# RaduAlexandru/permuto_sdf

Measured on AMD Instinct MI355X. Metric: ray-samples/sec (encode+MLP+composite), higher is better.
Workload: dtype f32 (MLP products on 2 fp16 operand pieces per fp32 value, fp32 accumulation; the 3-piece / 24-bit figure is value_fp32_equivalent_24bit)

## Files before the change

include/psdf.h:

```cpp
#ifndef PSDF_H
#define PSDF_H
#include <stdint.h>
#ifdef __cplusplus
extern "C" {
#endif

int64_t psdf_encode_convention(int which);
int psdf_encode_set_conventions(uint32_t hash_multiplier, int rank_tie_raises_later);

int psdf_encode_forward(int pos_dim, int nr_feat, int64_t N, int nr_levels, int capacity, const float* positions,
    const float* lattice, const float* scale_factor, const float* shifts, const float* window, int concat_points,
    float points_scaling, float* sliced, void* stream);

int psdf_encode_forward_mark(int pos_dim, int nr_feat, int64_t N, int nr_levels, int capacity, const float* positions,
    const float* lattice, const float* scale_factor, const float* shifts, const float* window, int concat_points,
    float points_scaling, float* sliced, unsigned char* touched_blocks, int block_rows_log2, void* stream);

int psdf_encode_backward(int pos_dim, int nr_feat, int64_t N, int nr_levels, int capacity, const float* positions,
    const float* lattice, const float* scale_factor, const float* shifts, const float* window, int concat_points,
    float points_scaling, const float* grad_sliced, float* grad_lattice, float* grad_positions, void* stream);

int64_t psdf_encode_backward_workspace_bytes(int pos_dim, int nr_feat, int64_t N, int nr_levels, int capacity);
int psdf_encode_backward_ws(int pos_dim, int nr_feat, int64_t N, int nr_levels, int capacity, const float* positions,
    const float* lattice, const float* scale_factor, const float* shifts, const float* window, int concat_points,
    float points_scaling, const float* grad_sliced, float* grad_lattice, float* grad_positions, void* workspace,
    int64_t workspace_bytes, void* stream);
int psdf_encode_backward_level_shares(int* counts, int max_levels);


int psdf_encode_double_backward(int pos_dim, int nr_feat, int64_t N, int nr_levels, int capacity, const float*
    positions, const float* lattice, const float* scale_factor, const float* shifts, const float* window, int
    concat_points, float points_scaling, const float* dd_positions, const float* grad_sliced, float* grad_lattice,
    float* grad_grad_sliced, void* stream);
int psdf_encode_double_backward_ws(int pos_dim, int nr_feat, int64_t N, int nr_levels, int capacity, const float* positions,
                                   const float* lattice, const float* scale_factor, const float* shifts, const float* window,
                                   int concat_points, float points_scaling, const float* dd_positions, const float* grad_sliced,
                                   float* grad_lattice, float* grad_grad_sliced, const float* grad_sliced_direct,
                                   void* workspace, int64_t workspace_bytes, void* stream);

int psdf_mlp_pack_f16(int n_layers, const int* dims, const float* const* weights, const float* const* biases, float* packed,
    void* stream);
int psdf_mlp_forward_f16(int n_layers, const int* dims, int64_t N, const float* X, const float* packed, float* Y, void* stream);

int psdf_mlp_forward_set_form(int waves);
int psdf_mlp_forward_last_form(void);

int psdf_neus_composite_forward(int nr_rays, const int* start_end, int equal, int fixed, int max_nr_samples, const float* sdf,
    const float* dirs, const float* gradients, const float* dt, const float* rgb, const float* inv_s, float cos_anneal_ratio,
    float* pred, float* bg, float* weights, void* stream);
int psdf_neus_composite_backward(int nr_rays, const int* start_end, int equal, int fixed, int max_nr_samples, int max_per_ray,
    const float* grad_pred, const float* grad_bg, const float* sdf, const float* dirs, const float* gradients, const float* dt,
    const float* rgb, const float* inv_s, float cos_anneal_ratio, int reference_compat, float* grad_sdf, float* grad_gradients,
    float* grad_rgb, float* grad_inv_s, void* stream);

int psdf_nerf_composite_forward(int nr_rays, const int* start_end, int equal, int fixed, int max_nr_samples, const float* raw_density,
                                const float* dt, const float* rgb, const float* fg_pred, const float* fg_bg, float* pred_bg,
                                float* pred, void* stream);
int psdf_nerf_composite_backward(int nr_rays, const int* start_end, int equal, int fixed, int max_nr_samples, int max_per_ray,
                                 const float* grad_pred, const float* fg_bg, const float* raw_density, const float* dt,
                                 const float* rgb, int reference_compat, float* grad_raw_density, float* grad_rgb,
                                 float* grad_fg_bg, void* stream);

int psdf_last_path(int family);
enum {
  PSDF_MLP_OP_FORWARD = 0,
  PSDF_MLP_OP_FORWARD_F16 = 1,
  PSDF_MLP_OP_FORWARD_WIDE_F16 = 2,
  PSDF_MLP_OP_BACKWARD = 3,
  PSDF_MLP_OP_BACKWARD_DATA = 4,
  PSDF_MLP_OP_BACKWARD_DATA_MASKED = 5,
  PSDF_MLP_OP_DOUBLE_BACKWARD = 6,
  PSDF_MLP_OP_DOUBLE_BACKWARD_PLUS = 7
};
int psdf_mlp_supported(int op, int n_layers, const int* dims);

int psdf_mlp_backward_split(int n_layers, const int* dims, int64_t N, const float* X, const float* const* weights,
    const float* const* biases, const float* dY, float* dX, float* const* dW, float* const* db, void* stream);

int psdf_mlp_backward_split_f16(int n_layers, const int* dims, int64_t N, const float* X, const float* const* weights,
    const float* const* biases, const float* dY, float* dX, float* const* dW, float* const* db, void* stream);
int psdf_mlp_backward_split_f16_form(void);
unsigned psdf_mlp_f16_range_events(void);

int psdf_mlp_forward_wide_f16(int n_layers, const int* dims, int64_t N, const float* X, const float* const* weights,
    const float* const* biases, float* Y, void* stream);
int psdf_mlp_backward_wide_form(void);
int psdf_mlp_backward_wide(int n_layers, const int* dims, int64_t N, const float* X, const float* const* weights,
    const float* const* biases, const float* dY, float* dX, float* const* dW, float* const* db, void* stream);

int psdf_lipshitz_normalize_forward(int out, int in, const float* W, const float* c, float* Wn, void* stream);
int psdf_lipshitz_normalize_backward(int out, int in, const float* W, const float* c, const float* grad_Wn, float* grad_W,
    float* grad_c, void* stream);
int psdf_lipshitz_normalize_forward_multi(int n_layers, const int* out, const int* in, const float* const* W, const float* const* c,
                                          float* const* Wn, void* stream);
int psdf_lipshitz_normalize_backward_multi(int n_layers, const int* out, const int* in, const float* const* W, const float* const* c,
                                           const float* const* grad_Wn, float* const* grad_W, float* const* grad_c, void* stream);

int psdf_neus_alpha_forward(int64_t N, const float* sdf, const float* dirs, const float* gradients, const float* dt,
    const float* inv_s, float cos_anneal_ratio, float* alpha, float* one_minus_alpha, void* stream);
int psdf_neus_alpha_backward(int64_t N, const float* grad_alpha, const float* sdf, const float* dirs, const float*
    gradients, const float* dt, const float* inv_s, float cos_anneal_ratio, float* grad_sdf, float* grad_gradients,
    float* grad_inv_s, void* stream);
int psdf_l1_loss(int64_t R, int C, const float* pred, const float* gt, const unsigned char* mask, float scale,
    float* loss, float* grad_pred, void* stream);
int psdf_eikonal_loss(int64_t N, const float* gradients, float scale, float* loss, float* grad_gradients, void* stream);
int psdf_normalize3(int64_t N, const float* x, const float* grad_y, float* out, void* stream);
int psdf_sigmoid_rows(int64_t N, int C, const float* x_fm, float* y, void* stream);
int psdf_sigmoid_rows_backward(int64_t N, int C, const float* grad_y, const float* y, float* grad_x_fm, void* stream);
int psdf_curvature_shift(int64_t N, const float* points, const float* gradients, const float* rand_directions, float
    epsilon, const float* grad_shifted, float* out, void* stream);
int psdf_curvature_loss(int64_t N, const float* gradients, const float* gradients_shifted, float scale, float* loss,
    float* grad_gradients, float* grad_gradients_shifted, void* stream);
int psdf_offsurface_loss(int64_t N, const float* sdf, float sharpness, float scale, float* loss, float* grad_sdf, void*
    stream);
int psdf_nerf_alpha_forward(int64_t N, const float* raw_density, const float* dt, float* alpha, float* one_minus_alpha,
    void* stream);
int psdf_nerf_alpha_backward(int64_t N, const float* raw_density, const float* dt, const float* grad_alpha, const float*
    grad_one_minus_alpha, float* grad_raw_density, void* stream);

int64_t psdf_mlp_packed_size(int n_layers, const int* dims);

int psdf_mlp_pack(int n_layers, const int* dims, const float* const* weights, const float* const* biases, float*
    packed, void* stream);

int psdf_mlp_forward(int n_layers, const int* dims, int64_t N, const float* X, const float* packed, float* Y, void*
    stream);

int psdf_encode_forward_masked(int pos_dim, int nr_feat, int64_t N, int nr_levels, int capacity, const float* positions,
    const float* lattice, const float* scale_factor, const float* shifts, const float* window, int concat_points, float
    points_scaling, const uint8_t* skip, float* sliced, void* stream);
int psdf_mlp_forward_masked(int n_layers, const int* dims, int64_t N, const float* X, const float* packed, const uint8_t*
    skip, float* Y, void* stream);
int psdf_mlp_backward_data_masked(int n_layers, const int* dims, int64_t N, const float* X, const float* const* weights,
    const float* const* biases, const float* dY, const uint8_t* skip, float* dX, void* stream);
int psdf_encode_backward_positions_masked(int pos_dim, int nr_feat, int64_t N, int nr_levels, int capacity, const float*
    positions, const float* lattice, const float* scale_factor, const float* shifts, const float* window, int
    concat_points, float points_scaling, const float* grad_sliced, const uint8_t* skip, float* grad_positions, void*
    stream);

int psdf_mlp_backward(int n_layers, const int* dims, int64_t N, const float* X, const float* const* weights, const
    float* const* biases, const float* dY, float* dX, float* const* dW, float* const* db, void* stream);

int psdf_mlp_double_backward(int n_layers, const int* dims, int64_t N, const float* X, const float* const* weights,
    const float* const* biases, const float* dY, const float* V, float* dX2, float* const* dW, float* const* db,
    void* stream);
int psdf_mlp_double_backward_plus(int n_layers, const int* dims, int64_t N, const float* X, const float* const* weights,
    const float* const* biases, const float* dY, const float* V, const float* dY2, float* dX2, float* const* dW,
    float* const* db, void* stream);

int psdf_encode_mlp_forward(int64_t N, int nr_levels, int capacity, const float* positions, const float* lattice,
    const float* scale_factor, const float* shifts, const float* window, int concat_points, float points_scaling,
    int n_layers, const int* dims, const float* packed, const uint8_t* skip, float* feat, float* Y, void* stream);

int psdf_adamw_step(int64_t n, float* param, const float* grad, float* exp_avg, float* exp_avg_sq, float lr, float
    beta1, float beta2, float eps, float weight_decay, int step, float grad_scale, void* stream);

int psdf_adamw_step_multi(int n_tensors, const int64_t* sizes, float* const* params, const float* const* grads, float*
    const* exp_avgs, float* const* exp_avg_sqs, float lr, float beta1, float beta2, float eps, float weight_decay, int
    step, float grad_scale, void* stream);

int psdf_adamw_step_blocks(int64_t n_blocks, int block_elems, float* param, float* grad, float* exp_avg, float*
// ... 193 lines not shown
```

permuto_sdf_amd/csrc/encode.hip:

```cpp
#include <cstdio>
#include <cstring>
#include <mutex>
#include <type_traits>
#include <vector>

#include "encode_device.h"
#include "encode_plan.h"

namespace {

template <int P, int F, bool PLAIN = false>
__global__ void __launch_bounds__(PSDF_BLOCK)
    encode_fwd_kernel(int64_t N, int L, uint32_t capacity, EncConv conv, const float* __restrict__ positions,
                      const float* __restrict__ lattice, const float* __restrict__ scale_factor,
                      const float* __restrict__ shifts, const float* __restrict__ window, float points_scaling,
                      int pad_points, const unsigned char* __restrict__ skip, float* __restrict__ sliced,
                      unsigned char* __restrict__ touched, int touch_shift, int blocks_per_level) {
  const int level = blockIdx.y;
  const int64_t ntiles = (N + PSDF_BLOCK - 1) / PSDF_BLOCK;
  for (int64_t tile = blockIdx.x; tile < ntiles; tile += gridDim.x) {
  const int64_t n = tile * PSDF_BLOCK + threadIdx.x;
  if (n >= N) continue;
  if (!PLAIN && skip && skip[n]) continue;
  float pos[P];
  load_pos<P>(positions, n, pos);
  if (level >= L) {
    const int e = level - L;
#pragma unroll
    for (int f = 0; f < F; f++) {
      const int d = e * F + f;
      float v = 0.f;
#pragma unroll
      for (int i = 0; i < P; i++)
        if (i == d) v = pos[i] * points_scaling;
      if (d < P || pad_points) sliced[((int64_t)level * F + f) * N + n] = v;
    }
    continue;
  }
  const float w = window[level];
  if (w == 0.f) {
#pragma unroll
    for (int f = 0; f < F; f++) sliced[((int64_t)level * F + f) * N + n] = 0.f;
    continue;
  }
  Simplex<P> s;
  compute_simplex<P>(pos, shifts + level * P, scale_factor + level * P, s, conv.tie_later);
  const float* __restrict__ table = lattice + (int64_t)level * capacity * F;
  uint32_t row[P + 1];
  vertex_rows<P>(s, capacity, row, conv.hash_c);
  if (!PLAIN && touched) {
#pragma unroll
    for (int r = 0; r <= P; r++) touched[(int64_t)level * blocks_per_level + (row[r] >> touch_shift)] = 1;
  }
  float fv[P + 1][F];
#pragma unroll
  for (int r = 0; r <= P; r++) {
    const char* tb = reinterpret_cast<const char*>(table);
    if (F == 2) {
      float2 t = *reinterpret_cast<const float2*>(tb + (row[r] * 8u));
      fv[r][0] = t.x;
      fv[r][F - 1] = t.y;
    } else {
#pragma unroll
      for (int f = 0; f < F; f++) fv[r][f] = *reinterpret_cast<const float*>(tb + (row[r] * (uint32_t)(F * 4) + (uint32_t)(f * 4)));
    }
  }
  float acc[F];
#pragma unroll
  for (int r = 0; r <= P; r++) {
    const float bw = s.bary[r] * w;
#pragma unroll
    for (int f = 0; f < F; f++) acc[f] = r == 0 ? fv[r][f] * bw : acc[f] + fv[r][f] * bw;
  }
#pragma unroll
  for (int f = 0; f < F; f++) sliced[((int64_t)level * F + f) * N + n] = acc[f];
  }
}


constexpr uint32_t SC_EMPTY = 0xFFFFFFFFu;
constexpr uint32_t Q_NONE = 0xFFFFFFFFu;
#if !defined(PSDF_ENC_QSPT)
#define PSDF_ENC_QSPT 2
#endif
constexpr int QUEUE_SPT = PSDF_ENC_QSPT;

__device__ __forceinline__ void lds_add_pair(float* p, float a, float b, int& hot) {
  if (hot == 0) {
    unsigned long long* q = reinterpret_cast<unsigned long long*>(p);
    unsigned long long old = *q;
#pragma unroll
    for (int it = 0; it < 4; it++) {
      const float x = __uint_as_float((uint32_t)old) + a;
      const float y = __uint_as_float((uint32_t)(old >> 32)) + b;
      const unsigned long long want = (unsigned long long)__float_as_uint(x) | ((unsigned long long)__float_as_uint(y) << 32);
      const unsigned long long prev = atomicCAS(q, old, want);
      if (prev == old) return;
      old = prev;
    }
    hot = 8;
  } else {
    hot--;
  }
  atomicAdd(p, a);
  atomicAdd(p + 1, b);
}

template <int F>
__device__ __forceinline__ bool combine_runs16(uint32_t key, float (&v)[F]) {
  constexpr int ROW_SHR = 0x110, ROW_SHL = 0x100;
  const int k = (int)key;
  const int kprev = __builtin_amdgcn_update_dpp(0, k, ROW_SHR | 1, 0xf, 0xf, true);
  const float joined = (kprev == k) ? 1.0f : 0.0f;
  float j = joined;
#define PSDF_SCAN_STEP(D)                                                                                        \
  {                                                                                                              \
    _Pragma("unroll") for (int i = 0; i < F; i++) v[i] = __builtin_fmaf(                                         \
        __int_as_float(__builtin_amdgcn_update_dpp(0, __float_as_int(v[i]), ROW_SHR | D, 0xf, 0xf, true)), j, v[i]); \
    j = j * __int_as_float(__builtin_amdgcn_update_dpp(0, __float_as_int(j), ROW_SHR | D, 0xf, 0xf, true));      \
  }
  PSDF_SCAN_STEP(1)
  PSDF_SCAN_STEP(2)
  PSDF_SCAN_STEP(4)
  PSDF_SCAN_STEP(8)
#undef PSDF_SCAN_STEP
  const int next_joined = __builtin_amdgcn_update_dpp(0, __float_as_int(joined), ROW_SHL | 1, 0xf, 0xf, true);
  return key != Q_NONE && next_joined == 0;
}

template <int F, int TOTAL = 8192>
struct ScatterCache {
  static constexpr int SC_SLOTS = TOTAL / F;
  uint32_t* tags;
  float* sums;
  int* stats;
  __device__ __forceinline__ void init(float* lds) {
    tags = reinterpret_cast<uint32_t*>(lds);
    sums = lds + SC_SLOTS;
    stats = reinterpret_cast<int*>(lds + SC_SLOTS + SC_SLOTS * F);
    for (int i = threadIdx.x; i < SC_SLOTS; i += blockDim.x) tags[i] = SC_EMPTY;
    for (int i = threadIdx.x; i < SC_SLOTS * F; i += blockDim.x) sums[i] = 0.f;
    if (threadIdx.x == 0) {
      stats[0] = 0;
      stats[1] = 0;
      stats[2] = 1;
    }
    __syncthreads();
  }
  __device__ __forceinline__ int add(uint32_t row, const float* v, int& hot) {
    const uint32_t slot = (row ^ (row >> 12)) & (SC_SLOTS - 1);
    uint32_t old = tags[slot];
    if (old == SC_EMPTY) old = atomicCAS(&tags[slot], SC_EMPTY, row);
    if (old == SC_EMPTY || old == row) {
      static_assert(F % 2 == 0, "pairs");
#pragma unroll
      for (int f = 0; f < F; f += 2) lds_add_pair(&sums[slot * F + f], v[f], v[f + 1], hot);
      return old == row ? 2 : 1;
    }
    return 0;
  }
  __device__ __forceinline__ void flush(float* __restrict__ table_grad) {
    __syncthreads();
    for (int i = threadIdx.x; i < SC_SLOTS; i += blockDim.x) {
      const uint32_t row = tags[i];
      if (row != SC_EMPTY) {
#pragma unroll
        for (int f = 0; f < F; f++) {
          const float v = sums[i * F + f];
          if (v != 0.f) atomicAdd(table_grad + (int64_t)row * F + f, v);
        }
      }
    }
  }
  static constexpr size_t bytes() { return (size_t)(SC_SLOTS + SC_SLOTS * F + 4) * 4; }
};

template <typename SC>
__device__ __forceinline__ bool cache_vote(SC& sc, int hits, int tries) {
  hits = (int)psdf::wave_sum((float)hits);
  tries = (int)psdf::wave_sum((float)tries);
  if (psdf::lane_id() == 0) {
    atomicAdd(&sc.stats[0], hits);
    atomicAdd(&sc.stats[1], tries);
  }
  __syncthreads();
  return sc.stats[0] * 8 >= sc.stats[1];
}

struct Queues {
  uint16_t* rows;
  float* vals;
  int* tails;
  int cap, np, shift;
};
using psdf::enc_plan::Q_MAX_PARTS;
constexpr int Q_LDS_INTS = 4 * Q_MAX_PARTS + 4;

struct LevelQueues {
  char* rows;
  char* vals;
  uint32_t mask;
};
template <int F>
__device__ __forceinline__ LevelQueues level_queues(const Queues& Q, int level) {
  const int64_t e = (int64_t)level * Q.np * Q.cap;
  return LevelQueues{reinterpret_cast<char*>(Q.rows + e), reinterpret_cast<char*>(Q.vals + e * F), (1u << Q.shift) - 1u};
}
template <int F>
__device__ __forceinline__ void queue_store(const LevelQueues& LQ, uint32_t o, uint32_t row, const float* v) {
  *reinterpret_cast<uint16_t*>(LQ.rows + (o * 2u)) = (uint16_t)(row & LQ.mask);
  if (F == 2) {
    *reinterpret_cast<float2*>(LQ.vals + (o * 8u)) = make_float2(v[0], v[F - 1]);
  } else {
#pragma unroll
    for (int f = 0; f < F; f++) *reinterpret_cast<float*>(LQ.vals + (o * (uint32_t)(F * 4) + (uint32_t)(f * 4))) = v[f];
  }
}

template <int NC, int F>
__device__ __forceinline__ void queue_push(const Queues& Q, int level, int* q_cnt, int* q_base,
                                           const uint32_t (&crow)[NC], const float (&cval)[NC][F],
                                           float* __restrict__ table_grad) {
  int* q_aux = q_base + Q_MAX_PARTS;
  const LevelQueues LQ = level_queues<F>(Q, level);
  if (threadIdx.x < Q.np) q_cnt[threadIdx.x] = 0;
  __syncthreads();
  int slot[NC];
#pragma unroll
// ... 578 lines not shown
  float sfl[P], shl[P];
#pragma unroll
  for (int i = 0; i < P; i++) {
    sfl[i] = scale_factor[level * P + i];
    shl[i] = shifts[level * P + i];
  }
  for (int64_t tile = blockIdx.x; tile < ntiles; tile += gridDim.x, iter++) {
    const int64_t n = tile * PSDF_BLOCK + threadIdx.x;
    if (n < N) {
      float u[P], pos[P];
      load_pos<P>(dd_positions, n, u);
      load_pos<P>(positions, n, pos);
      Simplex<P> s;
      compute_simplex<P>(pos, shl, sfl, s, conv.tie_later);
      float aE[P + 1];
#pragma unroll
      for (int j = 0; j <= P; j++) aE[j] = 0.f;
#pragma unroll
      for (int k = 0; k < P; k++) {
        const float us = u[k] * sfl[k];
#pragma unroll
        for (int j = 0; j <= k; j++) aE[j] = aE[j] + us;
        aE[k + 1] = aE[k + 1] - us * (float)(k + 1);
      }
      float q[P + 2];
#pragma unroll
      for (int k = 0; k <= P + 1; k++) q[k] = 0.f;
      const float invp = 1.0f / (P + 1);
#pragma unroll
      for (int i = 0; i <= P; i++) {
        const float t = aE[i] * invp;
#pragma unroll
        for (int k = 0; k <= P + 1; k++) {
          if (k == P - s.rank[i]) q[k] = q[k] + t;
          if (k == P + 1 - s.rank[i]) q[k] = q[k] - t;
        }
      }
      q[0] = q[0] + q[P + 1];
      float g[F], gg[F];
#pragma unroll
      for (int f = 0; f < F; f++) {
        g[f] = grad_sliced[((int64_t)level * F + f) * N + n];
        gg[f] = 0.f;
      }
      uint32_t rows[P + 1];
      vertex_rows<P>(s, capacity, rows, conv.hash_c);
#pragma unroll
      for (int r = 0; r <= P; r++) {
        const uint32_t row = rows[r];
        const float qw = q[r] * w;
        if (LATTICE) {
          float v[F];
#pragma unroll
          for (int f = 0; f < F; f++) v[f] = qw * g[f];
          bool absorbed = false;
          if (use_cache) {
            const int rc = sc.add(row, v, hot);
            absorbed = rc != 0;
            hits += (rc == 2);
            tries++;
          }
          if (!absorbed) {
#pragma unroll
            for (int f = 0; f < F; f++) atomicAdd(grad_lattice + tbase + (int64_t)row * F + f, v[f]);
          }
        }
#pragma unroll
        for (int f = 0; f < F; f++) gg[f] = gg[f] + qw * lattice[tbase + (int64_t)row * F + f];
      }
#pragma unroll
      for (int f = 0; f < F; f++) grad_grad_sliced[((int64_t)level * F + f) * N + n] = gg[f];
    }
    if (LATTICE && iter == 0) use_cache = cache_vote(sc, hits, tries);
  }
  if (LATTICE) sc.flush(grad_lattice + tbase);
}

inline int extra_levels(int P, int F, int concat) { return concat ? (P + F - 1) / F : 0; }
inline int pad_points(int concat) { return concat == PSDF_ENC_CONCAT_PSEUDO_LEVELS; }
inline bool concat_ok(int concat) { return concat >= PSDF_ENC_CONCAT_NONE && concat <= PSDF_ENC_CONCAT_APPEND; }

}

namespace psdf {
EncConv& enc_conv_state() {
  static EncConv c{(uint32_t)PSDF_ENC_HASH_MULTIPLIER, (uint32_t)PSDF_ENC_RANK_TIE_RAISES_LATER};
  return c;
}
}

namespace {
namespace plan = psdf::enc_plan;
using plan::env_int;
template <int V>
using int_c = std::integral_constant<int, V>;

template <class Fn>
int dispatch_pf(int pos_dim, int nr_feat, Fn&& fn) {
  if (pos_dim == 3 && nr_feat == 2) return fn(int_c<3>{}, int_c<2>{});
  if (pos_dim == 4 && nr_feat == 2) return fn(int_c<4>{}, int_c<2>{});
  if (pos_dim == 2 && nr_feat == 2) return fn(int_c<2>{}, int_c<2>{});
  if (pos_dim == 3 && nr_feat == 4) return fn(int_c<3>{}, int_c<4>{});
  return PSDF_ERR_UNSUPPORTED;
}

struct EncCall {
  int64_t N;
  int nr_levels, Lt, capacity;
  const float *positions, *lattice, *scale_factor, *shifts, *window;
  float points_scaling;
  int pad;
  hipStream_t stream;
};

bool enc_call(EncCall& c, int pos_dim, int nr_feat, int64_t N, int nr_levels, int capacity, const float* positions,
              const float* lattice, const float* scale_factor, const float* shifts, const float* window, int concat_points,
              float points_scaling, void* stream) {
  if (N < 0 || nr_levels <= 0 || capacity <= 0 || !positions || !lattice || !concat_ok(concat_points)) return false;
  c = EncCall{N, nr_levels, nr_levels + extra_levels(pos_dim, nr_feat, concat_points), capacity, positions, lattice,
              scale_factor, shifts, window, points_scaling, pad_points(concat_points), (hipStream_t)stream};
  return true;
}

template <class Kernel, class... Rest>
void launch_enc(Kernel kern, dim3 grid, size_t shm, const EncCall& c, Rest... rest) {
  hipLaunchKernelGGL(kern, grid, dim3(PSDF_BLOCK), shm, c.stream, c.N, c.nr_levels, (uint32_t)c.capacity, psdf::enc_conv_state(),
                     c.positions, c.lattice, c.scale_factor, c.shifts, c.window, c.points_scaling, rest...);
}

int launched(int rc) {
  if (rc != PSDF_OK) return rc;
  PSDF_LAUNCH_CHECK();
  return PSDF_OK;
}

int device_cus() {
  static int cus[64] = {};
  int dev = 0;
  if (hipGetDevice(&dev) != hipSuccess || dev < 0 || dev >= 64) return 256;
  if (cus[dev] == 0) {
    int n = 0;
    if (hipDeviceGetAttribute(&n, hipDeviceAttributeMultiprocessorCount, dev) != hipSuccess || n <= 0) n = 256;
    cus[dev] = n;
  }
  return cus[dev];
}

dim3 plain_grid(const EncCall& c) {
  static const int wg_cap_env = env_int("PSDF_ENC_BWD_WG_PER_LEVEL", 0);
  const unsigned wg_cap = wg_cap_env > 0 ? (unsigned)wg_cap_env : 512u, nb = psdf_blocks(c.N, PSDF_BLOCK);
  return dim3(nb < wg_cap ? nb : wg_cap, c.Lt);
}

template <int P, int F>
int launch_fwd(int_c<P>, int_c<F>, const EncCall& c, dim3 grid, const unsigned char* skip, float* sliced, unsigned char* touched,
               int touch_shift) {
  const int touch_blocks = (c.capacity + (1 << touch_shift) - 1) >> touch_shift;
  if (!skip && !touched)
    launch_enc(encode_fwd_kernel<P, F, true>, grid, 0, c, c.pad, skip, sliced, touched, touch_shift, touch_blocks);
  else
    launch_enc(encode_fwd_kernel<P, F, false>, grid, 0, c, c.pad, skip, sliced, touched, touch_shift, touch_blocks);
  return PSDF_OK;
}

int encode_forward_impl(int pos_dim, int nr_feat, int64_t N, int nr_levels, int capacity, const float* positions,
                        const float* lattice, const float* scale_factor, const float* shifts, const float* window,
                        int concat_points, float points_scaling, const unsigned char* skip, float* sliced, void* stream,
                        unsigned char* touched = nullptr, int touch_shift = 0) {
  EncCall c;
  if (N == 0) return PSDF_OK;
  if (!enc_call(c, pos_dim, nr_feat, N, nr_levels, capacity, positions, lattice, scale_factor, shifts, window, concat_points,
                points_scaling, stream) || !sliced)
    return PSDF_ERR_ARG;
  if ((int64_t)capacity * nr_feat * 4 > 0xffffffffll) return PSDF_ERR_UNSUPPORTED;
  dim3 grid(psdf_blocks(N, PSDF_BLOCK), c.Lt);
  static const int fwd_env = env_int("PSDF_ENC_FWD_WGS", -1);
  const int fwd_wgs = fwd_env >= 0 ? fwd_env : device_cus() * 8;
  if (fwd_wgs > 0 && (int)grid.x > fwd_wgs) grid.x = fwd_wgs;
  return launched(dispatch_pf(pos_dim, nr_feat, [&](auto p, auto f) {
    return launch_fwd(p, f, c, grid, skip, sliced, touched, touch_shift);
  }));
}

template <int P, int F, int POS_LPB>
void launch_bwd_pos_lpb(const EncCall& c, const float* grad_sliced, const unsigned char* skip, float* grad_positions, bool capturing) {
  static const bool force_atomics = env_int("PSDF_ENC_POS_ATOMICS", 0) != 0;
  const int groups = (c.Lt + POS_LPB - 1) / POS_LPB;
  static const size_t slab_cap = (size_t)plan::env_long("PSDF_ENC_POS_SLAB_MAX_MB", 256) << 20;
  const size_t slab_bytes = (size_t)groups * c.N * P * sizeof(float);
  const bool use_slabs = groups > 1 && !force_atomics && !capturing && slab_bytes <= slab_cap;
  float* slabs = use_slabs ? (float*)psdf::stream_scratch(slab_bytes, c.stream) : nullptr;
  const auto pos_kernel = [&](auto kern, float* out) {
    hipLaunchKernelGGL(kern, dim3(psdf_blocks(c.N, PSDF_BLOCK), groups), dim3(PSDF_BLOCK), 0, c.stream, c.N, c.nr_levels, c.Lt,
                       (uint32_t)c.capacity, psdf::enc_conv_state(), c.positions, c.lattice, c.scale_factor, c.shifts, c.window,
                       c.points_scaling, c.pad, grad_sliced, skip, out);
  };
  if (slabs) {
    pos_kernel(encode_bwd_pos_kernel<P, F, true, POS_LPB>, slabs);
    hipLaunchKernelGGL(encode_bwd_pos_reduce_kernel, dim3(psdf_blocks(c.N * P, PSDF_BLOCK)), dim3(PSDF_BLOCK), 0, c.stream,
                       c.N * P, P, groups, slabs, skip, grad_positions);
  } else {
    pos_kernel(encode_bwd_pos_kernel<P, F, false, POS_LPB>, grad_positions);
  }
}

template <int P, int F>
int launch_bwd_pos(int_c<P>, int_c<F>, const EncCall& c, const float* grad_sliced, const unsigned char* skip, float* grad_positions) {
  const bool capturing = psdf::stream_scratch(16, c.stream) == nullptr;
  if (capturing)
    launch_bwd_pos_lpb<P, F, 4>(c, grad_sliced, skip, grad_positions, true);
  else if (c.N >= ((int64_t)1 << 17))
    launch_bwd_pos_lpb<P, F, 2>(c, grad_sliced, skip, grad_positions, false);
  else
    launch_bwd_pos_lpb<P, F, 8>(c, grad_sliced, skip, grad_positions, false);
  return PSDF_OK;
}

plan::QueuePlan queue_plan(int pos_dim, int nr_feat, int64_t N, int nr_levels, int capacity) {
  static const int64_t min_n = plan::env_long("PSDF_ENC_QUEUE_MIN_N", (int64_t)1 << 13);
  static const int delta = env_int("PSDF_ENC_QUEUE_SLICE_LOG2_DELTA", 1);
  return plan::queue_plan(pos_dim, nr_feat, N, nr_levels, capacity, min_n, delta);
}
Queues queue_carve(void* ws, const plan::QueuePlan& p) {
  char* b = (char*)ws;
  return Queues{(uint16_t*)b, (float*)(b + p.rows_bytes), (int*)(b + p.rows_bytes + p.vals_bytes), p.cap, p.np, p.shift};
}
bool queue_begin(int pos_dim, int nr_feat, const EncCall& c, bool wanted, void* ws, int64_t ws_bytes, size_t also_zeroed, Queues& Q,
                 hipError_t& e) {
  const plan::QueuePlan p = (wanted && ws) ? queue_plan(pos_dim, nr_feat, c.N, c.nr_levels, c.capacity) : plan::QueuePlan{};
  if (p.bytes == 0 || ws_bytes < p.bytes) return false;
  Q = queue_carve(ws, p);
  e = hipMemsetAsync(Q.tails, 0, (size_t)c.nr_levels * Q.np * sizeof(int) + also_zeroed, c.stream);
  return true;
}

struct EncBalance {
  int levels = 0, total = 0, kind = 0, bucket = -1;
  const void* ident = nullptr;
  uint32_t gen = 0;
  uint64_t last_use = 0;
  std::vector<int> counts;
  uint32_t* times[2] = {nullptr, nullptr};
  int device = -1;
};
constexpr int BAL_STATES = 16;
std::mutex g_shares_mu;
std::vector<int> g_last_shares;

bool encode_balance(int nr_levels, int64_t N, int total, int64_t super_tiles, LevelPlan& lp, const void* ident, int kind) {
  static const bool off = env_int("PSDF_ENC_BWD_BALANCE", 1) == 0;
  static std::mutex mu;
  static EncBalance states[BAL_STATES];
  static uint64_t tick = 0;
  if (!plan::deal_eligible(off, nr_levels, total, N)) return false;
  std::lock_guard<std::mutex> lock(mu);
  const int bucket = plan::size_bucket(N);
  int device = -1;
  (void)hipGetDevice(&device);
  EncBalance* Bp = nullptr;
  for (auto& st_ : states)
    if (st_.times[0] && st_.ident == ident && st_.device == device && st_.kind == kind && st_.levels == nr_levels && st_.bucket == bucket &&
        st_.total == total)
      Bp = &st_;
  if (!Bp) {
    for (auto& st_ : states)
      if (!Bp || st_.last_use < Bp->last_use) Bp = &st_;
    if (!Bp->times[0]) {
      for (int i = 0; i < 2; i++) {
        void* h = nullptr;
        if (hipHostMalloc(&h, plan::BAL_MAX_WG * sizeof(uint32_t), hipHostMallocMapped) != hipSuccess || !h) {
          (void)hipGetLastError();
          if (i == 1) (void)hipHostFree(Bp->times[0]);
          Bp->times[0] = Bp->times[1] = nullptr;
          return false;
        }
        Bp->times[i] = (uint32_t*)h;
      }
    }
    memset(Bp->times[0], 0, plan::BAL_MAX_WG * sizeof(uint32_t));
    memset(Bp->times[1], 0, plan::BAL_MAX_WG * sizeof(uint32_t));
    Bp->levels = 0;
  }
  EncBalance& B = *Bp;
  B.last_use = ++tick;
  if (!B.times[0] || !B.times[1]) return false;
  const int cap = (int)(super_tiles < total ? super_tiles : total);
  if (B.levels != nr_levels || (int)B.counts.size() != nr_levels) {
    B.levels = nr_levels;
    B.kind = kind;
    B.ident = ident;
    B.device = device;
    B.bucket = bucket;
    B.total = total;
    B.counts = plan::first_deal(nr_levels, total);
  } else {
    plan::redeal_from_times(B.counts, B.times[B.gen & 1], B.gen, total, cap);
  }
  B.gen++;
  lp.n = nr_levels;
  lp.gen = B.gen;
  lp.times = B.times[B.gen & 1];
  const int at = plan::deal_layout(B.counts, cap, lp.first);
  std::lock_guard<std::mutex> l2(g_shares_mu);
  g_last_shares = B.counts;
  return at <= plan::BAL_MAX_WG;
}

template <class Kernel>
unsigned resident_round(Kernel kern, size_t shm, const EncCall& c, int deal_levels, int kind, LevelPlan& deal) {
  int per_cu = 0;
  const bool known = hipOccupancyMaxActiveBlocksPerMultiprocessor(&per_cu, kern, PSDF_BLOCK, shm) == hipSuccess && per_cu > 0;
  if (!known) (void)hipGetLastError();
  const int resident = known ? per_cu * device_cus() : 0;
  const int64_t tiles = plan::super_tiles(c.N, PSDF_BLOCK * QUEUE_SPT);
  deal = LevelPlan{};
  if (known && deal_levels > 0 && !encode_balance(deal_levels, c.N, resident, tiles, deal, c.lattice, kind)) deal = LevelPlan{};
  return plan::round_share(resident, c.nr_levels, tiles);
}

template <int F>
constexpr size_t binning_shm() { return ScatterCache<F, 4096>::bytes() + Q_LDS_INTS * sizeof(int); }

template <int P, int F, bool DBL>
unsigned launch_binning(const EncCall& c, int levels, const float* grad_sliced, float* grad_lattice, const Queues& Q,
                        const float* dd_positions, float* grad_grad_sliced, const float* grad_sliced2) {
  const auto kern = encode_bwd_kernel<P, F, true, false, true, DBL>;
  LevelPlan deal;
  const unsigned gx = resident_round(kern, binning_shm<F>(), c, levels, DBL ? 1 : 0, deal);
  launch_enc(kern, deal.n ? dim3(deal.first[deal.n]) : dim3(gx, levels), binning_shm<F>(), c, grad_sliced, grad_lattice,
             (float*)nullptr, Q, dd_positions, grad_grad_sliced, DBL ? c.pad : 0, grad_sliced2, deal);
  return gx;
}

template <int F>
int launch_queue_reduce(const EncCall& c, const Queues& Q, float* grad_lattice) {
  const size_t lds_b = (size_t)(1 << Q.shift) * F * sizeof(float);
  const hipError_t e =
      hipFuncSetAttribute((const void*)encode_bwd_reduce_kernel<F>, hipFuncAttributeMaxDynamicSharedMemorySize, (int)lds_b);
  if (e != hipSuccess) return (int)e;
  hipLaunchKernelGGL((encode_bwd_reduce_kernel<F>), dim3(Q.np, c.nr_levels), dim3(1024), lds_b, c.stream, (uint32_t)c.capacity, Q,
                     grad_lattice);
  return PSDF_OK;
}

#if defined(PSDF_ENC_PROFILE)
void enc_profile_report(const EncCall& c, int pos_dim, const Queues& Q, unsigned gx) {
  static int calls = 0;
  if (++calls != 8) return;
  (void)hipStreamSynchronize(c.stream);
  int prof[192];
  (void)hipMemcpy(prof, Q.tails + c.nr_levels * Q.np, sizeof(prof), hipMemcpyDeviceToHost);
  std::vector<int> tails((size_t)c.nr_levels * Q.np);
  (void)hipMemcpy(tails.data(), Q.tails, tails.size() * sizeof(int), hipMemcpyDeviceToHost);
  for (int l = 0; l < c.nr_levels; l++) {
    long long queued = 0;
    for (int q = 0; q < Q.np; q++) queued += tails[(size_t)l * Q.np + q];
    fprintf(stderr, "[enc-profile] level %2d: max %8d ticks, mean %8.0f ticks, cache kept by %d of %u workgroups, queued %lld of %lld "
            "contributions (%.1f %%)\n", l, prof[l], 64.0 * prof[64 + l] / gx, prof[128 + l], gx, queued,
            (long long)c.N * (pos_dim + 1), 100.0 * queued / ((double)c.N * (pos_dim + 1)));
  }
}
#endif

bool pos_fused() {
  static const bool on = env_int("PSDF_ENC_POS_FUSED", 0) != 0;
  return on;
}

template <int P, int F>
int launch_bwd(int_c<P> p, int_c<F> f, const EncCall& c, const float* grad_sliced, float* grad_lattice, float* grad_positions,
               const Queues* Q) {
  const float* const no_in = nullptr;
  float* const no_out = nullptr;
  constexpr size_t plain_shm = ScatterCache<F, 8192>::bytes() + Q_LDS_INTS * sizeof(int);
  if (!grad_lattice) return launch_bwd_pos(p, f, c, grad_sliced, nullptr, grad_positions);
  if (!Q) {
    if (grad_positions)
      launch_enc(encode_bwd_kernel<P, F, true, true, false>, plain_grid(c), plain_shm, c, grad_sliced, grad_lattice, grad_positions,
                 Queues{}, no_in, no_out, 0, no_in, LevelPlan{});
    else
      launch_enc(encode_bwd_kernel<P, F, true, false, false>, plain_grid(c), plain_shm, c, grad_sliced, grad_lattice, grad_positions,
                 Queues{}, no_in, no_out, 0, no_in, LevelPlan{});
    return PSDF_OK;
  }
  [[maybe_unused]] unsigned gx;
  if (grad_positions && pos_fused()) {
    const auto kern = encode_bwd_kernel<P, F, true, true, true>;
    LevelPlan none;
    gx = resident_round(kern, binning_shm<F>(), c, 0, 0, none);
    launch_enc(kern, dim3(gx, c.Lt), binning_shm<F>(), c, grad_sliced, grad_lattice, grad_positions, *Q, no_in, no_out, 0, no_in, none);
  } else {
    gx = launch_binning<P, F, false>(c, c.nr_levels, grad_sliced, grad_lattice, *Q, no_in, no_out, no_in);
    if (grad_positions) launch_bwd_pos(p, f, c, grad_sliced, nullptr, grad_positions);
  }
  const int rc = launch_queue_reduce<F>(c, *Q, grad_lattice);
#if defined(PSDF_ENC_PROFILE)
  if (rc == PSDF_OK) enc_profile_report(c, P, *Q, gx);
#endif
  return rc;
}

template <int P, int F>
int launch_dbl_queue(int_c<P>, int_c<F>, const EncCall& c, const float* dd_positions, const float* grad_sliced, float* grad_lattice,
                     float* grad_grad_sliced, const float* grad_sliced_direct, const Queues& Q) {
  launch_binning<P, F, true>(c, c.Lt, grad_sliced, grad_lattice, Q, dd_positions, grad_grad_sliced, grad_sliced_direct);
  return launch_queue_reduce<F>(c, Q, grad_lattice);
}

template <int P, int F>
int launch_dbl_plain(int_c<P>, int_c<F>, const EncCall& c, const float* dd_positions, const float* grad_sliced, float* grad_lattice,
                     float* grad_grad_sliced) {
  if (grad_lattice)
    launch_enc(encode_dbl_bwd_kernel<P, F, true>, plain_grid(c), ScatterCache<F>::bytes(), c, c.pad, dd_positions, grad_sliced,
               grad_lattice, grad_grad_sliced);
  else
    launch_enc(encode_dbl_bwd_kernel<P, F, false>, plain_grid(c), 0, c, c.pad, dd_positions, grad_sliced, grad_lattice,
               grad_grad_sliced);
  return PSDF_OK;
}

}

extern "C" {

int64_t psdf_encode_convention(int which) {
  switch (which) {
    case 0: return (int64_t)psdf::enc_conv_state().hash_c;
    case 1: return (int64_t)psdf::enc_conv_state().tie_later;
    case 2: return PSDF_ENC_SCALE_SQRT_TERM;
    case 3: return PSDF_ENC_SCALE_INV_STDDEV;
    case 4: return PSDF_ENC_CONCAT_DEFAULT_LAYOUT;
    default: return -1;
  }
}

int psdf_encode_set_conventions(uint32_t hash_multiplier, int rank_tie_raises_later) {
  if (hash_multiplier == 0u || (rank_tie_raises_later != 0 && rank_tie_raises_later != 1)) return PSDF_ERR_ARG;
  psdf::enc_conv_state() = EncConv{hash_multiplier, (uint32_t)rank_tie_raises_later};
  return PSDF_OK;
}

int psdf_encode_forward(int pos_dim, int nr_feat, int64_t N, int nr_levels, int capacity, const float* positions,
                        const float* lattice, const float* scale_factor, const float* shifts, const float* window,
                        int concat_points, float points_scaling, float* sliced, void* stream) {
  return encode_forward_impl(pos_dim, nr_feat, N, nr_levels, capacity, positions, lattice, scale_factor, shifts, window,
                             concat_points, points_scaling, nullptr, sliced, stream);
}

int psdf_encode_forward_masked(int pos_dim, int nr_feat, int64_t N, int nr_levels, int capacity, const float* positions,
                               const float* lattice, const float* scale_factor, const float* shifts, const float* window,
                               int concat_points, float points_scaling, const unsigned char* skip, float* sliced,
                               void* stream) {
  return encode_forward_impl(pos_dim, nr_feat, N, nr_levels, capacity, positions, lattice, scale_factor, shifts, window,
                             concat_points, points_scaling, skip, sliced, stream);
}

int psdf_encode_forward_mark(int pos_dim, int nr_feat, int64_t N, int nr_levels, int capacity, const float* positions,
                             const float* lattice, const float* scale_factor, const float* shifts, const float* window,
                             int concat_points, float points_scaling, float* sliced, unsigned char* touched_blocks,
                             int block_rows_log2, void* stream) {
  if (!touched_blocks || block_rows_log2 < 0 || block_rows_log2 > 20) return PSDF_ERR_ARG;
  return encode_forward_impl(pos_dim, nr_feat, N, nr_levels, capacity, positions, lattice, scale_factor, shifts, window,
                             concat_points, points_scaling, nullptr, sliced, stream, touched_blocks, block_rows_log2);
}

int64_t psdf_encode_backward_workspace_bytes(int pos_dim, int nr_feat, int64_t N, int nr_levels, int capacity) {
  return queue_plan(pos_dim, nr_feat, N, nr_levels, capacity).bytes;
}

int psdf_encode_backward_level_shares(int* counts, int max_levels) {
  std::lock_guard<std::mutex> lock(g_shares_mu);
  const int n = (int)g_last_shares.size();
  for (int l = 0; l < n && l < max_levels; l++) counts[l] = g_last_shares[l];
  return n;
}

int psdf_encode_backward_ws(int pos_dim, int nr_feat, int64_t N, int nr_levels, int capacity, const float* positions,
                            const float* lattice, const float* scale_factor, const float* shifts, const float* window,
                            int concat_points, float points_scaling, const float* grad_sliced, float* grad_lattice,
                            float* grad_positions, void* workspace, int64_t workspace_bytes, void* stream) {
  EncCall c;
  if (N == 0 || (!grad_lattice && !grad_positions)) return PSDF_OK;
  if (!enc_call(c, pos_dim, nr_feat, N, nr_levels, capacity, positions, lattice, scale_factor, shifts, window, concat_points,
                points_scaling, stream) || !grad_sliced)
    return PSDF_ERR_ARG;
  if (!grad_positions) c.Lt = nr_levels;
  Queues Q{};
  hipError_t e = hipSuccess;
#if defined(PSDF_ENC_PROFILE)
  const size_t profile_slots = 1024;
#else
  const size_t profile_slots = 0;
#endif
  const bool use_queue = queue_begin(pos_dim, nr_feat, c, grad_lattice, workspace, workspace_bytes, profile_slots, Q, e);
  if (e != hipSuccess) return (int)e;
  const int rc = dispatch_pf(pos_dim, nr_feat, [&](auto p, auto f) {
    return launch_bwd(p, f, c, grad_sliced, grad_lattice, grad_positions, use_queue ? &Q : nullptr);
  });
  if (rc == PSDF_OK) psdf::g_last_path[psdf::PATH_ENCODE_BWD] = use_queue ? 2 : (grad_lattice ? 1 : 3);
  return launched(rc);
}

int psdf_encode_backward(int pos_dim, int nr_feat, int64_t N, int nr_levels, int capacity, const float* positions,
                         const float* lattice, const float* scale_factor, const float* shifts, const float* window,
                         int concat_points, float points_scaling, const float* grad_sliced, float* grad_lattice,
                         float* grad_positions, void* stream) {
  return psdf_encode_backward_ws(pos_dim, nr_feat, N, nr_levels, capacity, positions, lattice, scale_factor, shifts,
                                 window, concat_points, points_scaling, grad_sliced, grad_lattice, grad_positions,
                                 nullptr, 0, stream);
}

int psdf_encode_backward_positions_masked(int pos_dim, int nr_feat, int64_t N, int nr_levels, int capacity,
                                          const float* positions, const float* lattice, const float* scale_factor,
                                          const float* shifts, const float* window, int concat_points, float points_scaling,
                                          const float* grad_sliced, const unsigned char* skip, float* grad_positions,
                                          void* stream) {
  EncCall c;
  if (N == 0) return PSDF_OK;
  if (!enc_call(c, pos_dim, nr_feat, N, nr_levels, capacity, positions, lattice, scale_factor, shifts, window, concat_points,
                points_scaling, stream) || !grad_sliced || !grad_positions)
    return PSDF_ERR_ARG;
  return launched(dispatch_pf(pos_dim, nr_feat, [&](auto p, auto f) {
    return launch_bwd_pos(p, f, c, grad_sliced, skip, grad_positions);
  }));
}

int psdf_encode_double_backward_ws(int pos_dim, int nr_feat, int64_t N, int nr_levels, int capacity,
                                   const float* positions, const float* lattice, const float* scale_factor,
                                   const float* shifts, const float* window, int concat_points, float points_scaling,
                                   const float* dd_positions, const float* grad_sliced, float* grad_lattice,
                                   float* grad_grad_sliced, const float* grad_sliced_direct, void* workspace,
                                   int64_t workspace_bytes, void* stream) {
  EncCall c;
  if (N == 0) return PSDF_OK;
  if (!enc_call(c, pos_dim, nr_feat, N, nr_levels, capacity, positions, lattice, scale_factor, shifts, window, concat_points,
                points_scaling, stream) || !dd_positions || !grad_sliced || (!grad_grad_sliced && !grad_lattice) ||
      (grad_sliced_direct && !grad_lattice))
    return PSDF_ERR_ARG;
  Queues Q{};
  hipError_t e = hipSuccess;
  if (queue_begin(pos_dim, nr_feat, c, grad_lattice, workspace, workspace_bytes, 0, Q, e)) {
    if (e != hipSuccess) return (int)e;
    return launched(dispatch_pf(pos_dim, nr_feat, [&](auto p, auto f) {
      return launch_dbl_queue(p, f, c, dd_positions, grad_sliced, grad_lattice, grad_grad_sliced, grad_sliced_direct, Q);
    }));
  }
  if (grad_sliced_direct) {
    const int rc = psdf_encode_backward_ws(pos_dim, nr_feat, N, nr_levels, capacity, positions, lattice, scale_factor, shifts,
                                           window, concat_points, points_scaling, grad_sliced_direct, grad_lattice, nullptr,
                                           nullptr, 0, stream);
    if (rc != PSDF_OK) return rc;
  }
  if (!grad_grad_sliced) {
    grad_grad_sliced = (float*)psdf::stream_scratch((size_t)c.Lt * nr_feat * N * sizeof(float), c.stream);
    if (!grad_grad_sliced) return PSDF_ERR_UNSUPPORTED;
  }
  return launched(dispatch_pf(pos_dim, nr_feat, [&](auto p, auto f) {
    return launch_dbl_plain(p, f, c, dd_positions, grad_sliced, grad_lattice, grad_grad_sliced);
  }));
}

int psdf_encode_double_backward(int pos_dim, int nr_feat, int64_t N, int nr_levels, int capacity,
                                const float* positions, const float* lattice, const float* scale_factor,
                                const float* shifts, const float* window, int concat_points, float points_scaling,
                                const float* dd_positions, const float* grad_sliced, float* grad_lattice,
                                float* grad_grad_sliced, void* stream) {
  return psdf_encode_double_backward_ws(pos_dim, nr_feat, N, nr_levels, capacity, positions, lattice, scale_factor, shifts,
                                        window, concat_points, points_scaling, dd_positions, grad_sliced, grad_lattice,
                                        grad_grad_sliced, nullptr, nullptr, 0, stream);
}

}
```

permuto_sdf_amd/csrc/encode_plan.h:

```cpp
#pragma once
#include <cstdint>
#include <cstdlib>
#include <vector>

namespace psdf {
namespace enc_plan {

inline int env_int(const char* name, int dflt) { const char* v = getenv(name); return v ? atoi(v) : dflt; }
inline long long env_long(const char* name, long long dflt) { const char* v = getenv(name); return v ? atoll(v) : dflt; }

constexpr int Q_MAX_PARTS = 64;

struct QueuePlan {
  int cap, np, shift;
  int64_t rows_bytes, vals_bytes, tails_bytes, bytes;
};

inline QueuePlan queue_plan(int pos_dim, int nr_feat, int64_t N, int nr_levels, int capacity, int64_t min_n, int slice_delta) {
  if (N < min_n) return QueuePlan{};
  const int base = (nr_feat <= 2) ? 14 : (nr_feat <= 4 ? 13 : 12);
  int shift = base - (slice_delta < 0 ? 0 : (slice_delta > 3 ? 3 : slice_delta));
  while (shift < base && ((capacity + (1 << shift) - 1) >> shift) > Q_MAX_PARTS) shift++;
  const int rpp = 1 << shift;
  const int np = (capacity + rpp - 1) / rpp;
  if (np > Q_MAX_PARTS || rpp * nr_feat * 4 > 128 * 1024) return QueuePlan{};
  const int64_t contrib = (int64_t)(pos_dim + 1) * N;
  const int64_t cap = (contrib / np) + (contrib / np) / 4 + 4096;
  if (cap > 0x7fffffff) return QueuePlan{};
  if ((int64_t)np * cap * (nr_feat * 4 > 2 ? nr_feat * 4 : 2) > 0xffffffffll) return QueuePlan{};
  const auto round256 = [](int64_t b) { return (b + 255) & ~(int64_t)255; };
  const int64_t entries = (int64_t)nr_levels * np * cap;
  QueuePlan p{(int)cap, np, shift, round256(entries * 2), round256(entries * nr_feat * 4), round256((int64_t)nr_levels * np * 4), 0};
  p.bytes = p.rows_bytes + p.vals_bytes + p.tails_bytes + 1024;
  return p;
}

inline int64_t super_tiles(int64_t N, int tile) { return (N + tile - 1) / tile; }

inline unsigned round_share(int resident, int nr_levels, int64_t tiles) {
  int64_t gx = resident > 0 ? (int64_t)resident / nr_levels : 128;
  if (gx > tiles) gx = tiles;
  return (unsigned)(gx < 1 ? 1 : gx);
}

constexpr int BAL_MAX_WG = 8192, BAL_MIN_PER_LEVEL = 4, BAL_MAX_LEVELS = 40;

inline int size_bucket(int64_t N) {
  int bucket = 0;
  for (int64_t v = N; v > 1; v >>= 1) bucket += 4;
  const int64_t top = (int64_t)1 << (bucket / 4);
  return bucket + (int)(((N - top) * 4) / top);
}

inline bool deal_eligible(bool switched_off, int nr_levels, int total, int64_t N) {
  return !(switched_off || nr_levels > BAL_MAX_LEVELS || total > BAL_MAX_WG || total < nr_levels * BAL_MIN_PER_LEVEL ||
           N < ((int64_t)1 << 18));
}

inline std::vector<int> first_deal(int nr_levels, int total) { return std::vector<int>((size_t)nr_levels, total / nr_levels); }

inline void redeal(std::vector<int>& counts, const double* work, int total, int cap) {
  const int n = (int)counts.size();
  double sum = 0.0;
  for (int l = 0; l < n; l++) sum += work[l];
  if (!(sum > 0.0)) return;
  int used = 0;
  for (int l = 0; l < n; l++) {
    int c = (int)(0.5 * counts[l] + 0.5 * total * work[l] / sum + 0.5);
    c = c < BAL_MIN_PER_LEVEL ? BAL_MIN_PER_LEVEL : (c > cap ? cap : c);
    counts[l] = c;
    used += c;
  }
  while (used > total) {
    int big = 0;
    for (int l = 1; l < n; l++)
      if (counts[l] > counts[big]) big = l;
    if (counts[big] <= BAL_MIN_PER_LEVEL) break;
    counts[big]--;
    used--;
  }
}

inline bool redeal_from_times(std::vector<int>& counts, const volatile uint32_t* times, uint32_t gen, int total, int cap) {
  std::vector<double> work(counts.size(), 0.0);
  int id = 0;
  for (size_t l = 0; l < counts.size(); l++)
    for (int b = 0; b < counts[l]; b++, id++) {
      const uint32_t v = times[id];
      if ((v >> 24) != (gen & 255u) || (v & 0xFFFFFFu) == 0u) return false;
      work[l] += (double)(v & 0xFFFFFFu);
    }
  redeal(counts, work.data(), total, cap);
  return true;
}

inline int deal_layout(std::vector<int>& counts, int cap, uint16_t* first) {
  int at = 0;
  for (size_t l = 0; l < counts.size(); l++) {
    if (counts[l] > cap) counts[l] = cap;
    if (counts[l] < 1) counts[l] = 1;
    first[l] = (uint16_t)at;
    at += counts[l];
  }
  first[counts.size()] = (uint16_t)at;
  return at;
}

}
}
```

Baseline: 1.002 billion.

## Pair coarse and fine lattice levels per workgroup in forward encode

Result: faster. 1.020 billion (median of 6 runs) (+1.7%).

```diff
diff --git a/include/psdf.h b/include/psdf.h
--- a/include/psdf.h
+++ b/include/psdf.h
@@ -7,6 +7,8 @@
 
 int64_t psdf_encode_convention(int which);
 int psdf_encode_set_conventions(uint32_t hash_multiplier, int rank_tie_raises_later);
+
+int psdf_encode_set_forward_pairs(int pairs);
 
 int psdf_encode_forward(int pos_dim, int nr_feat, int64_t N, int nr_levels, int capacity, const float* positions,
     const float* lattice, const float* scale_factor, const float* shifts, const float* window, int concat_points,
diff --git a/permuto_sdf_amd/csrc/encode.hip b/permuto_sdf_amd/csrc/encode.hip
--- a/permuto_sdf_amd/csrc/encode.hip
+++ b/permuto_sdf_amd/csrc/encode.hip
@@ -8,6 +8,96 @@
 #include "encode_plan.h"
 
 namespace {
+
+struct FwdArgs {
+  int64_t N;
+  int L;
+  uint32_t capacity;
+  EncConv conv;
+  const float *lattice, *scale_factor, *shifts, *window;
+  float points_scaling;
+  int pad_points;
+  float* sliced;
+  unsigned char* touched;
+  int touch_shift, blocks_per_level;
+};
+
+template <int P, int F>
+struct FwdGather {
+  float fv[P + 1][F];
+  float bw[P + 1];
+};
+
+template <int P, int F>
+__device__ __forceinline__ bool fwd_level_flat(const FwdArgs& A, int level, int64_t n, const float (&pos)[P]) {
+  if (level >= A.L) {
+    const int e = level - A.L;
+#pragma unroll
+    for (int f = 0; f < F; f++) {
+      const int d = e * F + f;
+      float v = 0.f;
+#pragma unroll
+      for (int i = 0; i < P; i++)
+        if (i == d) v = pos[i] * A.points_scaling;
+      if (d < P || A.pad_points) A.sliced[((int64_t)level * F + f) * A.N + n] = v;
+    }
+    return true;
+  }
+  if (A.window[level] == 0.f) {
+#pragma unroll
+    for (int f = 0; f < F; f++) A.sliced[((int64_t)level * F + f) * A.N + n] = 0.f;
+    return true;
+  }
+  return false;
+}
+
+template <int P, int F, bool PLAIN>
+__device__ __forceinline__ void fwd_level_gather(const FwdArgs& A, int level, int64_t n, const float (&pos)[P], FwdGather<P, F>& g) {
+  const float w = A.window[level];
+  Simplex<P> s;
+  compute_simplex<P>(pos, A.shifts + level * P, A.scale_factor + level * P, s, A.conv.tie_later);
+  const float* __restrict__ table = A.lattice + (int64_t)level * A.capacity * F;
+  uint32_t row[P + 1];
+  vertex_rows<P>(s, A.capacity, row, A.conv.hash_c);
+  if (!PLAIN && A.touched) {
+#pragma unroll
+    for (int r = 0; r <= P; r++) A.touched[(int64_t)level * A.blocks_per_level + (row[r] >> A.touch_shift)] = 1;
+  }
+#pragma unroll
+  for (int r = 0; r <= P; r++) {
+    const char* tb = reinterpret_cast<const char*>(table);
+    if (F == 2) {
+      float2 t = *reinterpret_cast<const float2*>(tb + (row[r] * 8u));
+      g.fv[r][0] = t.x;
+      g.fv[r][F - 1] = t.y;
+    } else {
+#pragma unroll
+      for (int f = 0; f < F; f++) g.fv[r][f] = *reinterpret_cast<const float*>(tb + (row[r] * (uint32_t)(F * 4) + (uint32_t)(f * 4)));
+    }
+  }
+#pragma unroll
+  for (int r = 0; r <= P; r++) g.bw[r] = s.bary[r] * w;
+}
+
+template <int P, int F>
+__device__ __forceinline__ void fwd_level_finish(const FwdArgs& A, int level, int64_t n, const FwdGather<P, F>& g) {
+  float acc[F];
+#pragma unroll
+  for (int r = 0; r <= P; r++) {
+#pragma unroll
+    for (int f = 0; f < F; f++) acc[f] = r == 0 ? g.fv[r][f] * g.bw[r] : acc[f] + g.fv[r][f] * g.bw[r];
+  }
+#pragma unroll
+  for (int f = 0; f < F; f++) A.sliced[((int64_t)level * F + f) * A.N + n] = acc[f];
+}
+
+template <int P, int F, bool PLAIN>
+__device__ __forceinline__ void fwd_level(const FwdArgs& A, int level, int64_t n, const float (&pos)[P]) {
+  if (fwd_level_flat<P, F>(A, level, n, pos)) return;
+  FwdGather<P, F> g;
+  fwd_level_gather<P, F, PLAIN>(A, level, n, pos, g);
+  fwd_level_finish<P, F>(A, level, n, g);
+}
 
 template <int P, int F, bool PLAIN = false>
 __global__ void __launch_bounds__(PSDF_BLOCK)
@@ -16,64 +106,77 @@
                       const float* __restrict__ shifts, const float* __restrict__ window, float points_scaling,
                       int pad_points, const unsigned char* __restrict__ skip, float* __restrict__ sliced,
                       unsigned char* __restrict__ touched, int touch_shift, int blocks_per_level) {
+  const FwdArgs A{N, L, capacity, conv, lattice, scale_factor, shifts, window, points_scaling, pad_points, sliced, touched,
+                  touch_shift, blocks_per_level};
   const int level = blockIdx.y;
   const int64_t ntiles = (N + PSDF_BLOCK - 1) / PSDF_BLOCK;
   for (int64_t tile = blockIdx.x; tile < ntiles; tile += gridDim.x) {
-  const int64_t n = tile * PSDF_BLOCK + threadIdx.x;
-  if (n >= N) continue;
-  if (!PLAIN && skip && skip[n]) continue;
-  float pos[P];
-  load_pos<P>(positions, n, pos);
-  if (level >= L) {
-    const int e = level - L;
-#pragma unroll
-    for (int f = 0; f < F; f++) {
-      const int d = e * F + f;
-      float v = 0.f;
-#pragma unroll
-      for (int i = 0; i < P; i++)
-        if (i == d) v = pos[i] * points_scaling;
-      if (d < P || pad_points) sliced[((int64_t)level * F + f) * N + n] = v;
-    }
-    continue;
-  }
-  const float w = window[level];
-  if (w == 0.f) {
-#pragma unroll
-    for (int f = 0; f < F; f++) sliced[((int64_t)level * F + f) * N + n] = 0.f;
-    continue;
-  }
-  Simplex<P> s;
-  compute_simplex<P>(pos, shifts + level * P, scale_factor + level * P, s, conv.tie_later);
-  const float* __restrict__ table = lattice + (int64_t)level * capacity * F;
-  uint32_t row[P + 1];
-  vertex_rows<P>(s, capacity, row, conv.hash_c);
-  if (!PLAIN && touched) {
-#pragma unroll
-    for (int r = 0; r <= P; r++) touched[(int64_t)level * blocks_per_level + (row[r] >> touch_shift)] = 1;
-  }
-  float fv[P + 1][F];
-#pragma unroll
-  for (int r = 0; r <= P; r++) {
-    const char* tb = reinterpret_cast<const char*>(table);
-    if (F == 2) {
-      float2 t = *reinterpret_cast<const float2*>(tb + (row[r] * 8u));
-      fv[r][0] = t.x;
-      fv[r][F - 1] = t.y;
-    } else {
-#pragma unroll
-      for (int f = 0; f < F; f++) fv[r][f] = *reinterpret_cast<const float*>(tb + (row[r] * (uint32_t)(F * 4) + (uint32_t)(f * 4)));
-    }
-  }
-  float acc[F];
-#pragma unroll
-  for (int r = 0; r <= P; r++) {
-    const float bw = s.bary[r] * w;
-#pragma unroll
-    for (int f = 0; f < F; f++) acc[f] = r == 0 ? fv[r][f] * bw : acc[f] + fv[r][f] * bw;
-  }
-#pragma unroll
-  for (int f = 0; f < F; f++) sliced[((int64_t)level * F + f) * N + n] = acc[f];
+    const int64_t n = tile * PSDF_BLOCK + threadIdx.x;
+    if (n >= N) continue;
+    if (!PLAIN && skip && skip[n]) continue;
+    float pos[P];
+    load_pos<P>(positions, n, pos);
+    fwd_level<P, F, PLAIN>(A, level, n, pos);
+  }
+}
+
+template <class T>
+__device__ __forceinline__ T per_tile(T v) {
+  asm volatile("" : "+s"(v));
+  return v;
+}
+
+template <int P, int F, bool PLAIN = false>
+__global__ void __launch_bounds__(PSDF_BLOCK)
+    encode_fwd_pair_kernel(int64_t N, int L, uint32_t capacity, EncConv conv, const float* __restrict__ positions,
+                           const float* __restrict__ lattice, const float* __restrict__ scale_factor,
+                           const float* __restrict__ shifts, const float* __restrict__ window, float points_scaling,
+                           int pad_points, const unsigned char* __restrict__ skip, float* __restrict__ sliced,
+                           unsigned char* __restrict__ touched, int touch_shift, int blocks_per_level,
+                           psdf::enc_plan::FwdSlots slots) {
+  const FwdArgs A{N, L, capacity, conv, lattice, scale_factor, shifts, window, points_scaling, pad_points, sliced, touched,
+                  touch_shift, blocks_per_level};
+  const int la = slots.a[blockIdx.y], lb = slots.b[blockIdx.y];
+  const bool two = lb != psdf::enc_plan::FWD_SLOT_NONE;
+  const bool together = two && la < L && lb < L && window[la] != 0.f && window[lb] != 0.f;
+  const uint32_t ntiles = (uint32_t)((N + PSDF_BLOCK - 1) / PSDF_BLOCK);
+  if (together) {
+    for (uint32_t tile = blockIdx.x; tile < ntiles; tile += gridDim.x) {
+      const int64_t n = (int64_t)tile * PSDF_BLOCK + threadIdx.x;
+      if (n >= N) continue;
+      if (!PLAIN) {
+        const unsigned char* sk = per_tile(skip);
+        if (sk && sk[n]) continue;
+      }
+      float pos[P];
+      load_pos<P>(positions, n, pos);
+      const int xa = per_tile(la), xb = per_tile(lb);
+      FwdArgs B = A;
+      B.capacity = per_tile(A.capacity);
+      B.conv.hash_c = per_tile(A.conv.hash_c);
+      B.conv.tie_later = per_tile(A.conv.tie_later);
+      if (!PLAIN) B.touched = per_tile(A.touched);
+      FwdGather<P, F> ga, gb;
+      fwd_level_gather<P, F, PLAIN>(B, xa, n, pos, ga);
+      fwd_level_gather<P, F, PLAIN>(B, xb, n, pos, gb);
+      fwd_level_finish<P, F>(A, xa, n, ga);
+      fwd_level_finish<P, F>(A, xb, n, gb);
+    }
+  } else {
+    for (int k = 0; k < (two ? 2 : 1); k++) {
+      const int level = k ? lb : la;
+      for (uint32_t tile = blockIdx.x; tile < ntiles; tile += gridDim.x) {
+        const int64_t n = (int64_t)tile * PSDF_BLOCK + threadIdx.x;
+        if (n >= N) continue;
+        if (!PLAIN) {
+          const unsigned char* sk = per_tile(skip);
+          if (sk && sk[n]) continue;
+        }
+        float pos[P];
+        load_pos<P>(positions, n, pos);
+        fwd_level<P, F, PLAIN>(A, per_tile(level), n, pos);
+      }
+    }
   }
 }
 
@@ -958,14 +1061,27 @@
   return dim3(nb < wg_cap ? nb : wg_cap, c.Lt);
 }
 
+int& fwd_pairs_setting() {
+  static int v = env_int("PSDF_ENC_FWD_PAIRS", -1);
+  return v;
+}
+
 template <int P, int F>
 int launch_fwd(int_c<P>, int_c<F>, const EncCall& c, dim3 grid, const unsigned char* skip, float* sliced, unsigned char* touched,
-               int touch_shift) {
+               int touch_shift, const plan::FwdSlots& slots) {
   const int touch_blocks = (c.capacity + (1 << touch_shift) - 1) >> touch_shift;
-  if (!skip && !touched)
+  const bool plain = !skip && !touched;
+  if (slots.n > 0) {
+    grid.y = (unsigned)slots.n;
+    if (plain)
+      launch_enc(encode_fwd_pair_kernel<P, F, true>, grid, 0, c, c.pad, skip, sliced, touched, touch_shift, touch_blocks, slots);
+    else
+      launch_enc(encode_fwd_pair_kernel<P, F, false>, grid, 0, c, c.pad, skip, sliced, touched, touch_shift, touch_blocks, slots);
+  } else if (plain) {
     launch_enc(encode_fwd_kernel<P, F, true>, grid, 0, c, c.pad, skip, sliced, touched, touch_shift, touch_blocks);
-  else
+  } else {
     launch_enc(encode_fwd_kernel<P, F, false>, grid, 0, c, c.pad, skip, sliced, touched, touch_shift, touch_blocks);
+  }
   return PSDF_OK;
 }
 
@@ -983,8 +1099,12 @@
   static const int fwd_env = env_int("PSDF_ENC_FWD_WGS", -1);
   const int fwd_wgs = fwd_env >= 0 ? fwd_env : device_cus() * 8;
   if (fwd_wgs > 0 && (int)grid.x > fwd_wgs) grid.x = fwd_wgs;
+  const int want = fwd_pairs_setting();
+  const int pairs = want < 0 ? plan::forward_pairs_default(nr_levels, N) : want;
+  const bool pairable = pairs > 0 && (N + PSDF_BLOCK - 1) / PSDF_BLOCK <= 0xffffffffll;
+  const plan::FwdSlots slots = pairable ? plan::forward_slots(nr_levels, c.Lt, pairs) : plan::FwdSlots{};
   return launched(dispatch_pf(pos_dim, nr_feat, [&](auto p, auto f) {
-    return launch_fwd(p, f, c, grid, skip, sliced, touched, touch_shift);
+    return launch_fwd(p, f, c, grid, skip, sliced, touched, touch_shift, slots);
   }));
 }
 
@@ -1246,6 +1366,12 @@
   return PSDF_OK;
 }
 
+int psdf_encode_set_forward_pairs(int pairs) {
+  if (pairs < -1) return PSDF_ERR_ARG;
+  fwd_pairs_setting() = pairs;
+  return PSDF_OK;
+}
+
 int psdf_encode_forward(int pos_dim, int nr_feat, int64_t N, int nr_levels, int capacity, const float* positions,
                         const float* lattice, const float* scale_factor, const float* shifts, const float* window,
                         int concat_points, float points_scaling, float* sliced, void* stream) {
diff --git a/permuto_sdf_amd/csrc/encode_plan.h b/permuto_sdf_amd/csrc/encode_plan.h
--- a/permuto_sdf_amd/csrc/encode_plan.h
+++ b/permuto_sdf_amd/csrc/encode_plan.h
@@ -106,5 +106,39 @@
   return at;
 }
 
+constexpr int FWD_MAX_SLOTS = 42;
+constexpr uint8_t FWD_SLOT_NONE = 0xFF;
+struct FwdSlots {
+  int n;
+  uint8_t a[FWD_MAX_SLOTS];
+  uint8_t b[FWD_MAX_SLOTS];
+};
+
+inline FwdSlots forward_slots(int L, int Lt, int pairs) {
+  FwdSlots s{};
+  if (L < 1 || Lt < L || Lt >= (int)FWD_SLOT_NONE) return s;
+  if (pairs < 0) pairs = 0;
+  if (pairs > L / 2) pairs = L / 2;
+  if (Lt - pairs > FWD_MAX_SLOTS) return s;
+  int at = 0;
+  for (int i = 0; i < pairs; i++, at++) {
+    s.a[at] = (uint8_t)i;
+    s.b[at] = (uint8_t)(L - 1 - i);
+  }
+  for (int l = pairs; l < Lt; l++) {
+    if (l < L && l >= L - pairs) continue;
+    s.a[at] = (uint8_t)l;
+    s.b[at] = FWD_SLOT_NONE;
+    at++;
+  }
+  s.n = at;
+  return s;
+}
+
+inline int forward_pairs_default(int L, int64_t N) {
+  (void)N;
+  return L / 2;
+}
+
 }
 }
```
